# B3zaleel/draco-sharp

Hardware: AMD Instinct MI355X
Metric: decoded_meshes_per_sec (higher is better)
Workload: dtype int32

## Files before the change

draco-sharp_amd/csrc/dsa_kernels.h:

```cpp
#pragma once
#include <hip/hip_runtime.h>
#include <stdint.h>

#include "dsa_common.h"
#include "dsa_locate.h"
#include "dsa_needs.h"
#ifdef DSA_EXPERIMENTS
#include "dsa_lanes.h"
#else
#define LN_FLAG_SYMBOLS 1u
#define LN_FLAG_PREDICT 2u
#define LN_FLAG_OCT 8u
namespace dsa { namespace lanes {
__device__ __forceinline__ bool ln_sym_eligible(const AttrDesc &, const MeshLayout &, uint32_t, uint32_t) { return false; }
__device__ __forceinline__ bool ln_oct_eligible(const AttrDesc &, uint32_t) { return false; }
} }
#endif

#ifndef DSA_CHAIN_PRIO
#define DSA_CHAIN_PRIO 3
#endif

namespace dsa {

// ... 1376 lines not shown
        }
      }
      bool went_left = false;
      if (!went_right) {
        if (bits & 4u) {
          if (bits & 8u) { --sp; TPROF(5); break; }
          corner = lc;
          went_left = true;
        } else {
          if (bits & 8u) { corner = rc; went_right = true; }
          else {
            if (sp >= stack_cap) TR_FAIL(304);
            if (lane == 0) { stack[sp - 1] = lc; stack[sp] = rc; }
            ++sp;
            TPROF(5);
            break;
          }
        }
      }
      if (went_right && have2) { have_rec = true; have_state = true; c_v = c2_v; c_rc = c2_rc; c_lc = c2_lc; c_bits = c2_bits; }
      else if (have_kids && went_right) { have_rec = true; c_v = kr_v; c_rc = kr_rc; c_lc = kr_lc; }
      else if (have_kids && went_left) { have_rec = true; c_v = kl_v; c_rc = kl_rc; c_lc = kl_lc; }
      have2 = false;
      TPROF(5);
    }
    if (failed) break;
  }
  if (failed) return;
  if (lane == 0 && !position) { if (count != expect) fail(D, ST_INVALID, 305); }
  if (lane == 0 && position) {
    D->num_entries = count;
    D->dbg[5] = n_fail; D->dbg[6] = (uint32_t)(clk() - t_start);
    D->dbg[16] = (uint32_t)r_start; D->dbg[17] = (uint32_t)(realclk() - r_start);
    D->dbg[7] = n_run; D->dbg[8] = n_run_faces; D->dbg[9] = n_scalar; D->dbg[3] = n_fast;
#ifdef DSA_TRAV_PROFILE
    for (int i = 0; i < 5; ++i) D->dbg[10 + (i < 3 ? i : i + 5)] = (uint32_t)(tp_acc[i] >> 4);
    D->dbg[0] = (uint32_t)(tp_acc[5] >> 4); D->dbg[1] = np_fast_hit; D->dbg[2] = np_dep; D->dbg[4] = np_head; D->dbg[13] = np_hist; D->dbg[14] = np_lin; D->dbg[15] = np_hand;
    D->dbg[16] = np_pairs1; D->dbg[17] = np_pairs2;
#endif
    if (count != expect) fail(D, ST_INVALID, 305);
  }
  if ((fuse_operands & 1u) && count == expect) {
    WAIT_VM0();
    __threadfence_block();
    uint32_t *para = io.para;
    for (uint32_t p0 = 0; p0 < count; p0 += 4 * WAVE) {
      uint32_t en[4], ep[4], eo[4];
#pragma unroll
      for (int u = 0; u < 4; ++u) {
        const uint32_t p = p0 + u * WAVE + lane;
        para_operands_flat<CP>(p < count ? p : 0u, frec, d2c, v2d, F, NV, en[u], ep[u], eo[u]);
      }
#pragma unroll
      for (int u = 0; u < 4; ++u) {
        const uint32_t p = p0 + u * WAVE + lane;
        if (p < count) { Triple t; t.a = en[u]; t.b = ep[u]; t.c = eo[u]; *(Triple *)(para + 3 * (size_t)p) = t; }
      }
    }
  }
  if (position && !D->seam_fast && count == expect && NV) {
    WAIT_VM0();
    __threadfence_block();
    const uint32_t *vrank = (const uint32_t *)(arena + L.vrank);
    const uint32_t na = uni(D->num_attributes), npts = uni(D->num_points);
    for (uint32_t v0 = 0; v0 < NV; v0 += 4 * WAVE) {
      int32_t e[4];
      uint32_t point[4];
#pragma unroll
      for (int u = 0; u < 4; ++u) {
        const uint32_t v = v0 + u * WAVE + lane, vc = v < NV ? v : NV - 1;
        e[u] = v < NV ? v2d[vc] : -1;
        point[u] = vrank[vc];
      }
#pragma unroll
      for (int u = 0; u < 4; ++u)
        if (e[u] >= 0 && point[u] < npts)
          for (uint32_t ai = 0; ai < na; ++ai) ((uint32_t *)(arena + L.map[ai]))[point[u]] = (uint32_t)e[u];
    }
  }
#undef TR_FAIL
#undef VISIT_SCALAR
#undef TPROF
#undef TCOUNT
#undef TADD
#undef fA_before
#undef fB_before
#undef fR_before
#undef fL_before
#undef fLA_before
#undef flA
#undef flB
#undef TR_MARKS
}

__global__ __launch_bounds__(WAVE) void k_traverse(uint8_t *arena, const MeshLayout *layouts, MeshDesc *descs, uint32_t n, uint32_t fuse_operands) {
  __shared__ unsigned long long sh_tf[TR_SLOTS], sh_tv[TR_SLOTS];
  __shared__ uint32_t sh_hist[TR_HIST_WORDS];
  for (uint32_t i = threadIdx.x; i < TR_SLOTS; i += WAVE) { sh_tf[i] = 0; sh_tv[i] = 0; }
  if (threadIdx.x < TR_HIST_WORDS) sh_hist[threadIdx.x] = 0;
  __syncthreads();
  __builtin_amdgcn_s_setprio(DSA_CHAIN_PRIO);
  const uint32_t mesh = blockIdx.x;
  if (mesh >= n) return;
  if (status_of(&descs[mesh]) != ST_OK) return;
  const TravIO io = trav_position(arena, layouts[mesh], &descs[mesh]);
  if (layouts[mesh].rec_compact) traverse_wave<true>(arena, layouts[mesh], &descs[mesh], io, fuse_operands, sh_tf, sh_tv, sh_hist);
  else traverse_wave<false>(arena, layouts[mesh], &descs[mesh], io, fuse_operands, sh_tf, sh_tv, sh_hist);
}

extern __shared__ __attribute__((aligned(16))) uint32_t sh_chain[];
__global__ __launch_bounds__(WAVE, 8) void k_chain(uint8_t *arena, const MeshLayout *layouts, MeshDesc *descs, uint32_t n, uint32_t fuse_operands) {
  uint32_t *sh = sh_chain;
  static_assert(CN_LDS_WORDS * 4 >= 2 * TR_SLOTS * 8 + TR_HIST_WORDS * 4, "the traversal's tables reuse the connectivity's LDS");
  __builtin_amdgcn_s_setprio(DSA_CHAIN_PRIO);
  const uint32_t mesh = blockIdx.x;
  if (mesh >= n) return;
  const MeshLayout &L = layouts[mesh];
  MeshDesc *D = &descs[mesh];
  const bool compact = uni(L.rec_compact) != 0;
  uint32_t *sh_rec = sh + CN_STAGE * 8, *sh_win = sh_rec + CN_REC_BLOCKS * 64 * 2, *sh_ctx = sh_win + CN_WIN;
  if (!compact) connectivity_wave<false, false>(arena, L, D, sh, sh_rec, sh_win, sh_ctx);
  else if (uni((uint32_t)D->traversal_type) == 2u) connectivity_wave<true, true>(arena, L, D, sh, sh_rec, sh_win, sh_ctx);
  else connectivity_wave<true, false>(arena, L, D, sh, sh_rec, sh_win, sh_ctx);
  __builtin_amdgcn_fence(__ATOMIC_SEQ_CST, "agent");
  __syncthreads();
  unsigned long long *sh_tf = (unsigned long long *)sh, *sh_tv = sh_tf + TR_SLOTS;
  uint32_t *sh_hist = sh + 2 * TR_SLOTS * 2;
  for (uint32_t i = threadIdx.x; i < TR_SLOTS; i += WAVE) { sh_tf[i] = 0; sh_tv[i] = 0; }
  if (threadIdx.x < TR_HIST_WORDS) sh_hist[threadIdx.x] = 0;
  __syncthreads();
  if (status_of(D) != ST_OK) return;
  const TravIO io = trav_position(arena, L, D);
  if (compact) traverse_wave<true>(arena, L, D, io, fuse_operands, sh_tf, sh_tv, sh_hist);
  else traverse_wave<false>(arena, L, D, io, fuse_operands, sh_tf, sh_tv, sh_hist);
  if ((fuse_operands & 1u) && (fuse_operands & 8u) && status_of(D) == ST_OK) {
    const uint32_t na = uni(D->num_attributes);
    for (uint32_t ai = 0; ai < na && ai < DSA_MAX_ATT; ++ai) late_handoff(arena, L, D, ai, PW_FLAG | LATE_HANDOFF, 2u);
  }
}



__device__ __forceinline__ void rans_decode_wave(MeshDesc *D, const uint8_t *stream, uint32_t stream_len, const AttrDesc &a, uint32_t num_values,
                                 uint32_t *out, uint32_t *lds_cum, uint32_t *symtab) {
  const uint32_t lane = lane_id();
  const uint32_t nsym = symtab ? a.num_distinct : a.num_symbols;
  const uint32_t P = a.precision_bits, precision = 1u << P, l_base = precision * 4;
  if (lane == 0) {
    Rd r(stream, stream_len, a.off_table);
    if (symtab) {
      uint32_t k = 0;
      bool ok = true;
      for (uint32_t i = 0; i < a.num_symbols && ok; ++i) {
        const uint32_t pd = r.u8(), token = pd & 3u;
        if (token == 3u) { const uint32_t offset = pd >> 2; if (i + offset >= a.num_symbols) ok = false; i += offset; }
        else {
          uint32_t pr = pd >> 2;
          for (uint32_t j = 0; j < token; ++j) pr |= r.u8() << (8 * (j + 1) - 2);
          if (pr) { if (k >= nsym) ok = false; else { lds_cum[k] = pr; symtab[k] = i; ++k; } }
        }
      }
      if (!ok || !r.ok || k != nsym) fail(D, ST_INVALID, 400);
    } else if (!read_prob_table(r, nsym, lds_cum)) fail(D, ST_INVALID, 400);
  }
  WAIT_VM0();
  __syncthreads();
  if (status_of(D) != ST_OK) return;
  uint32_t carry = 0;
  for (uint32_t b0 = 0; b0 < nsym; b0 += WAVE) {
    uint32_t i = b0 + lane;
    uint32_t pr = i < nsym ? lds_cum[i] : 0u;
    uint32_t tot;
    uint32_t ex = wave_excl_scan(pr, &tot);
    if (i < nsym) lds_cum[i] = carry + ex;
    carry += tot;
  }
  if (carry != precision) { if (lane == 0) fail(D, ST_INVALID, 401); return; }
  const uint32_t nblocks = (nsym + WAVE - 1) / WAVE;
  for (uint32_t i = nsym + lane; i < nblocks * WAVE + 1; i += WAVE) lds_cum[i] = precision;
  __syncthreads();
  uint32_t coarse = (lane < nblocks) ? lds_cum[lane * WAVE] : precision;
  uint32_t fine0 = lds_cum[lane];
  const uint8_t *buf = stream + a.off_rans;
  uint32_t x, off;
  {
    uint32_t st = 0, o = 0;
    bool ok = rans_init(buf, a.size_rans, l_base, &st, &o);
    if (!ok) { if (lane == 0) fail(D, ST_INVALID, 402); return; }
    x = uni(st); off = uni(o);
  }
  const uintptr_t base_addr = (uintptr_t)buf;
  const uint32_t mis = (uint32_t)(base_addr & 3u);
  const uint32_t *abuf = (const uint32_t *)(base_addr - mis);
  uint32_t chunk = 0xFFFFFFFFu, W = 0;
  const uint32_t mask = precision - 1;
  uint32_t mine = 0;
  for (uint32_t i = 0; i < num_values; ++i) {
    while (x < l_base && off > 0) {
      --off;
      uint32_t q = off + mis;
      uint32_t ch = q >> 8;
      if (ch != chunk) { chunk = ch; W = abuf[(size_t)ch * 64 + lane]; }
      uint32_t byte = (rdlane(W, (q & 255u) >> 2) >> ((q & 3u) * 8)) & 0xFFu;
      x = (x << 8) | byte;
    }
    uint32_t rem = x & mask;
    uint32_t s, cs, nx;
    if (nblocks == 1) {
      uint32_t j = (uint32_t)__popcll(__ballot(fine0 <= rem)) - 1u;
      cs = rdlane(fine0, j);
      nx = (j < 63) ? rdlane(fine0, j + 1) : precision;
      s = j;
    } else {
      uint32_t b = (uint32_t)__popcll(__ballot(coarse <= rem)) - 1u;
      uint32_t v = lds_cum[b * WAVE + lane];
      uint32_t j = (uint32_t)__popcll(__ballot(v <= rem)) - 1u;
      cs = rdlane(v, j);
      nx = (j < 63) ? rdlane(v, j + 1) : rdlane(coarse, b + 1);
      s = b * WAVE + j;
    }
    x = (nx - cs) * (x >> P) + rem - cs;
    if ((i & 63u) == lane) mine = s;
    if ((i & 63u) == 63u) out[i - 63u + lane] = mine;
  }
  uint32_t tail = num_values & 63u;
  if (tail && lane < tail) out[num_values - tail + lane] = mine;
  if (symtab) {
    WAIT_VM0();
    __syncthreads();
    for (uint32_t i = lane; i < num_values; i += WAVE) out[i] = symtab[out[i]];
  }
}

__device__ __forceinline__ void rans_decode_serial(MeshDesc *D, const uint8_t *stream, uint32_t stream_len, const AttrDesc &a, uint32_t num_values,
                                   uint32_t *out, uint32_t *cum ) {
  if (threadIdx.x != 0) return;
  const uint32_t nsym = a.num_symbols, P = a.precision_bits, precision = 1u << P, l_base = precision * 4;
  Rd r(stream, stream_len, a.off_table);
  if (!read_prob_table(r, nsym, cum)) { fail(D, ST_INVALID, 410); return; }
  uint32_t c = 0;
  for (uint32_t i = 0; i < nsym; ++i) { uint32_t pr = cum[i]; cum[i] = c; c += pr; if (c > precision) break; }
  if (c != precision) { fail(D, ST_INVALID, 411); return; }
  cum[nsym] = precision;
  const uint8_t *buf = stream + a.off_rans;
  uint32_t x, off;
  if (!rans_init(buf, a.size_rans, l_base, &x, &off)) { fail(D, ST_INVALID, 412); return; }
  for (uint32_t i = 0; i < num_values; ++i) {
    while (x < l_base && off > 0) x = (x << 8) | buf[--off];
    uint32_t rem = x & (precision - 1);
    uint32_t lo = 0, hi = nsym;
    while (hi - lo > 1) { uint32_t mid = (lo + hi) >> 1; if (cum[mid] <= rem) lo = mid; else hi = mid; }
    uint32_t cs = cum[lo];
    x = (cum[lo + 1] - cs) * (x >> P) + rem - cs;
    out[i] = lo;
  }
}

typedef uint32_t v32u __attribute__((ext_vector_type(32)));

#define SYM_EARLY_FUSE 0x400u
__device__ __forceinline__ void predict_wave(uint8_t *arena, const MeshLayout &L, MeshDesc *D, uint32_t ai, uint32_t phase, uint32_t flags);
__device__ __forceinline__ void predict_wrap_attribute(uint8_t *arena, const MeshLayout &L, MeshDesc *D, uint32_t ai, uint32_t phase, uint32_t flags);
__device__ __forceinline__ void finalize_attribute(uint8_t *arena, const MeshLayout &L, const MeshDesc *D, uint32_t ai, uint32_t phase, uint32_t flags, uint32_t tid, uint32_t stride);
__device__ __forceinline__ void early_tail(uint8_t *arena, const MeshLayout &L, MeshDesc *D, uint32_t ai, uint32_t flags) {
  if (!(flags & SYM_EARLY_FUSE) || D->general) return;
  const AttrDesc &a = D->att[ai];
  if (att_is_late(a)) return;
  WAIT_VM0();
  __threadfence_block();
  __syncthreads();
  if (status_of(D) != ST_OK) return;
  predict_wrap_attribute(arena, L, D, ai, 0u, flags);
  predict_wave(arena, L, D, ai, 0u, flags);
  WAIT_VM0();
  __threadfence_block();
  __syncthreads();
  if (status_of(D) != ST_OK) return;
  finalize_attribute(arena, L, D, ai, 0u, flags, lane_id(), WAVE);
  if (lane_id() == 0) D->att[ai].early_done = 1;
}

__device__ __forceinline__ void late_handoff(uint8_t *arena, const MeshLayout &L, MeshDesc *D, uint32_t ai, uint32_t flags, uint32_t bit) {
  if (!(flags & LATE_HANDOFF) || D->general) return;
  AttrDesc &a = D->att[ai];
  if (!wrap_fast_ok(a, flags) || !att_is_late(a) || att_behind_tables(a) || a.pred_kind != 1) return;
  __builtin_amdgcn_fence(__ATOMIC_RELEASE, "agent");
  __syncthreads();
  uint32_t old = 0;
  if (lane_id() == 0) old = __hip_atomic_fetch_or(&a.late_ready, bit, __ATOMIC_ACQ_REL, __HIP_MEMORY_SCOPE_AGENT);
  old = uni(old);
  if (!(old & (3u ^ bit))) return;
  __builtin_amdgcn_fence(__ATOMIC_ACQUIRE, "agent");
  if (status_of(D) != ST_OK) return;
  predict_wrap_attribute(arena, L, D, ai, 1u, flags);
  WAIT_VM0();
  __syncthreads();
  if (lane_id() == 0) a.late_ready = 7u;
}

#define REG_ATTR 0
#define REG_TAGS 1
#define REG_VLIST 2
#define REG_SCRATCH_BYTES (4096u * 6u + REG_MAX_SYMS * 4u)
template <int MODE>
__device__ __forceinline__ void reg_decode_stream(uint8_t *arena, const MeshLayout &L, MeshDesc *D, uint32_t ai, uint32_t flags) {
  constexpr bool TAGS = MODE == REG_TAGS, VLIST = MODE == REG_VLIST;
  AttrDesc &a = D->att[VLIST ? 0u : ai];
  uint8_t *scratch;
  uint32_t st_off_table = a.off_table, st_off_rans = a.off_rans, st_size_rans = a.size_rans, st_nsym = a.num_symbols;
  uint32_t st_values = a.num_entries * (TAGS ? 1u : (uint32_t)a.nc_portable);
  uint32_t *out = (uint32_t *)(arena + L.work[VLIST ? 0u : ai]);
  if (VLIST) {
    st_values = D->val_count[ai];
    if (st_values == 0 || D->val_prec[ai] != 12 || D->val_nsym[ai] > 64) return;
    if ((uint64_t)L.rec_compact * 16ull * D->num_faces < 6ull * REG_SCRATCH_BYTES) return;
    st_off_table = D->val_off_table[ai]; st_off_rans = D->val_off_rans[ai]; st_size_rans = D->val_size_rans[ai]; st_nsym = D->val_nsym[ai];
    uint32_t before = 0;
    for (uint32_t k = 0; k < ai; ++k) before += D->val_count[k];
    if ((uint64_t)before + st_values > 3ull * D->num_faces) return;
    out = (uint32_t *)(arena + L.faces) + before;
    scratch = arena + L.frec + (size_t)ai * REG_SCRATCH_BYTES;
  } else if (TAGS) {
    if (a.source != SRC_TAGGED || a.tags_done || a.num_symbols > LOC_MAX_TAGS || a.num_distinct <= 1 || a.num_entries == 0) return;
    const uint64_t slots = ((uint64_t)a.num_entries * 4 + 15) & ~15ull;
    if ((uint64_t)L.work_cap[ai] * 4 < slots + REG_SCRATCH_BYTES) return;
    scratch = arena + L.work[ai] + slots;
  } else {
    if (lanes::ln_sym_eligible(a, L, ai, flags)) return;
    if (sym_filtered(a, flags)) return;
    if (!sym_reg_eligible(a, L, ai)) return;
    scratch = arena + L.out[ai];
  }
  const uint8_t *stream = arena + L.stream;
  uint32_t *slot_tab = (uint32_t *)scratch;
  uint16_t *slot_sym = (uint16_t *)(scratch + 4096 * 4);
  uint32_t *lds = (uint32_t *)(scratch + 4096 * 6);
  const uint32_t lane = lane_id();
  const uint32_t nsym = uni(st_nsym);
  const uint32_t num_values = uni(st_values);
  if (num_values == 0) return;
  if (lane == 0) {
    Rd r(stream, L.stream_len, st_off_table);
    if (!read_prob_table(r, nsym, lds)) fail(D, ST_INVALID, 400);
  }
  __syncthreads();
  if (status_of(D) != ST_OK) return;
  uint32_t carry = 0, one_at = DSA_INVALID;
  bool over = false;
  for (uint32_t b0 = 0; b0 < REG_MAX_SYMS; b0 += WAVE) {
    uint32_t i = b0 + lane;
    uint32_t pr = i < nsym ? lds[i] : 0u;
    if (pr > 4095) { over = true; one_at = i; }
    uint32_t tot;
    uint32_t ex = wave_excl_scan(pr, &tot);
    lds[i] = (pr << 12) | ((carry + ex) & 4095u);
    carry += tot;
    if (carry > 4096) over = true;
  }
  if (VLIST && carry == 4096 && __ballot(over)) {
    uint32_t st = 0, o = 0;
    if (!rans_init(stream + st_off_rans, st_size_rans, 16384, &st, &o)) { if (lane == 0) fail(D, ST_INVALID, 402); return; }
    const uint32_t one = (uint32_t)__builtin_ctzll(__ballot(one_at != DSA_INVALID));
    const uint32_t sym = rdlane(one_at, one);
    for (uint32_t i = lane; i < num_values; i += WAVE) out[i] = sym;
    WAIT_VM0();
    __syncthreads();
    if (lane == 0) atomicOr(&D->val_lists_done, 1u << ai);
    return;
  }
  if (__ballot(over) || carry != 4096) { if (lane == 0) fail(D, carry != 4096 ? ST_INVALID : ST_NOTIMPL, 401); return; }
  __syncthreads();
  for (uint32_t sy = lane; sy < nsym; sy += WAVE) {
    const uint32_t e = lds[sy], f = e >> 12, c = e & 4095u;
    for (uint32_t j = 0; j < f; ++j) { slot_tab[c + j] = f | (j << 16); slot_sym[c + j] = (uint16_t)sy; }
  }
  WAIT_VM0();
  __syncthreads();
  v32u tab_lo, tab_hi;
#pragma unroll
  for (int k = 0; k < 32; ++k) { tab_lo[k] = slot_tab[k * WAVE + lane]; tab_hi[k] = slot_tab[(k + 32) * WAVE + lane]; }
  const uint8_t *buf = stream + st_off_rans;
  uint32_t x, off;
  {
    uint32_t st = 0, o = 0;
    bool ok = rans_init(buf, st_size_rans, 16384, &st, &o);
    if (!ok) { if (lane == 0) fail(D, ST_INVALID, 402); return; }
    x = uni(st); off = uni(o);
  }
  const uint32_t mis = (uint32_t)((L.stream + st_off_rans) & 3u);
  const uint32_t *abuf = (const uint32_t *)(arena + (L.stream + st_off_rans - mis));
  uint32_t chunk = 0x7FFFFFFFu, W = 0;
  uint32_t mine = 0;
  WAIT_VM0();
  uint64_t P = (uint64_t)x << 32;
  uint32_t rc = 0;
  uint32_t dl = 0;
  bool exhausted = false;
  for (uint32_t i0 = 0; i0 < num_values; i0 += WAVE) {
    const uint32_t cnt = uni(num_values - i0 < WAVE ? num_values - i0 : WAVE);
    uint32_t j = 0;
    while (j < cnt) {
      if (!exhausted) {
        {
          uint32_t k6, va, vf;
          uint32_t js = uni(j);
          asm volatile(
              " s_getpc_b64 s[22:23]\n"
              "Lupc%=:\n"
              " s_mul_i32 %[k6], %[j], Lus1_%=-Lus0_%=\n"
              " s_add_u32 s22, s22, Lus0_%=-Lupc%=\n"
              " s_addc_u32 s23, s23, 0\n"
              " s_add_u32 s22, s22, %[k6]\n"
              " s_addc_u32 s23, s23, 0\n"
              " s_set_gpr_idx_on s22, gpr_idx(SRC1)\n"
              " s_setpc_b64 s[22:23]\n"
              ".irp J,0,1,2,3,4,5,6,7,8,9,10,11,12,13,14,15,16,17,18,19,20,21,22,23,24,25,26,27,28,29,30,31,32,33,34,35,36,37,38,39,40,41,42,43,44,45,46,47,48,49,50,51,52,53,54,55,56,57,58,59,60,61,62,63\n"
              "Lus\\J\\()_%=:\n"
              " s_cmpk_lt_u32 s21, 0x4000\n"
              " s_cbranch_scc1 Lur\\J\\()_%=\n"
              "Lok\\J\\()_%=:\n"
              " s_bfe_u32 %[k6], s21, 0x60006\n"
              " s_set_gpr_idx_idx %[k6]\n"
              " v_lshrrev_b32_e64 %[vf], 12, s21\n"
              " v_mul_u32_u24_sdwa %[va], %[vf], v16 dst_sel:DWORD dst_unused:UNUSED_PAD src0_sel:DWORD src1_sel:WORD_0\n"
              " v_add_u32_sdwa %[va], %[va], v16 dst_sel:DWORD dst_unused:UNUSED_PAD src0_sel:DWORD src1_sel:WORD_1\n"
              " v_writelane_b32 %[mine], s21, \\J\n"
              " v_readlane_b32 s21, %[va], s21\n"
              ".endr\n"
              " s_movk_i32 %[j], 64\n"
              " s_branch Luend%=\n"
              ".irp J,0,1,2,3,4,5,6,7,8,9,10,11,12,13,14,15,16,17,18,19,20,21,22,23,24,25,26,27,28,29,30,31,32,33,34,35,36,37,38,39,40,41,42,43,44,45,46,47,48,49,50,51,52,53,54,55,56,57,58,59,60,61,62,63\n"
              "Lur\\J\\()_%=:\n"
              " s_sub_u32 %[rc], %[rc], 1\n"
              " s_cbranch_scc1 Lue\\J\\()_%=\n"
              " s_lshl_b64 s[20:21], s[20:21], 8\n"
              " s_cmpk_lt_u32 s21, 0x4000\n"
              " s_cbranch_scc0 Lok\\J\\()_%=\n"
              " s_branch Lur\\J\\()_%=\n"
              "Lue\\J\\()_%=:\n"
              " s_cmp_lt_u32 %[off], 4\n"
              " s_cbranch_scc1 Lsl\\J\\()_%=\n"
              " s_sub_u32 %[dl], %[dl], 1\n"
              " s_cbranch_scc1 Lsl\\J\\()_%=\n"
              " v_readlane_b32 s20, %[W], %[dl]\n"
              " s_sub_u32 %[off], %[off], 4\n"
              " s_mov_b32 %[rc], 3\n"
              " s_lshl_b64 s[20:21], s[20:21], 8\n"
              " s_cmpk_lt_u32 s21, 0x4000\n"
              " s_cbranch_scc0 Lok\\J\\()_%=\n"
              " s_branch Lur\\J\\()_%=\n"
              "Lsl\\J\\()_%=:\n"
              " s_movk_i32 %[j], \\J\n"
              " s_branch Luempty%=\n"
              ".endr\n"
              "Luempty%=:\n"
              " s_mov_b32 %[rc], 0\n"
              "Luend%=:\n"
              " s_set_gpr_idx_off\n"
              : "+{s[20:21]}"(P), [rc] "+s"(rc), [j] "+s"(js), [mine] "+v"(mine), [k6] "=&s"(k6), [va] "=&v"(va), [vf] "=&v"(vf),
                [off] "+s"(off), [dl] "+s"(dl)
              : "{v[16:47]}"(tab_lo), "{v[48:79]}"(tab_hi), [W] "v"(W)
              : "vcc", "scc", "s22", "s23");
          j = js;
        }
        if (j < cnt) {
          if (off == 0) exhausted = true;
          else {
            const uint32_t end = off + mis;
            const uint32_t d = (end - 1) >> 2, r = end - 4 * d, ch = d >> 6;
            if (ch != chunk) { chunk = ch; W = abuf[(size_t)ch * 64 + lane]; WAIT_VM0(); }
            const uint32_t res = rdlane(W, d & 63u) << (8 * (4 - r));
            rc = uni(r < off ? r : off);
            off -= rc;
            dl = uni(d & 63u);
            P = (P & 0xFFFFFFFF00000000ull) | res;
          }
        }
      } else {
        const uint32_t xs = uni((uint32_t)(P >> 32));
        mine = (lane == j) ? xs : mine;
        const uint32_t k5 = (xs >> 6) & 31u, l6 = xs & 63u;
        const uint32_t e0 = rdlane(tab_lo[k5], l6), e1 = rdlane(tab_hi[k5], l6);
        const uint32_t e = (xs & 2048u) ? e1 : e0;
        P = (uint64_t)((e & 0xFFFFu) * (xs >> 12) + (e >> 16)) << 32;
        ++j;
      }
    }
    if (lane < cnt) out[i0 + lane] = mine;
  }
  WAIT_VM0();
  __syncthreads();
  if (VLIST) {
    for (uint32_t i = lane; i < num_values; i += WAVE) out[i] = slot_sym[out[i] & 4095u];
    WAIT_VM0();
    __syncthreads();
    if (lane == 0) atomicOr(&D->val_lists_done, 1u << ai);
    return;
  }
  if (TAGS) {
    uint8_t *tags = arena + L.out[ai];
    uint64_t bits = 0;
    uint32_t worst = 0;
    const uint32_t nc = a.nc_portable;
    for (uint32_t i = lane; i < num_values; i += WAVE) {
      const uint32_t v = slot_sym[out[i] & 4095u];
      tags[i] = (uint8_t)v;
      bits += (uint64_t)v * nc;
      worst = v > worst ? v : worst;
    }
    for (int d = 32; d >= 1; d >>= 1) {
      bits += ((uint64_t)(uint32_t)__shfl_xor((int)(uint32_t)(bits >> 32), d, WAVE) << 32) | (uint32_t)__shfl_xor((int)(uint32_t)bits, d, WAVE);
      const uint32_t w2 = (uint32_t)__shfl_xor((int)worst, d, WAVE);
      worst = w2 > worst ? w2 : worst;
    }
    WAIT_VM0();
    __syncthreads();
    if (lane == 0) { a.table = (bits & 0x00FFFFFFFFFFFFFFull) | ((uint64_t)(worst > 255u ? 255u : worst) << 56); a.tags_done = 1; }
    return;
  }
  const bool positive = a.have_scheme && (a.pred_transform == 2 || a.pred_transform == 3);
  for (uint32_t i = lane; i < num_values; i += WAVE) {
    uint32_t v = slot_sym[out[i] & 4095u];
    out[i] = positive ? v : ((v & 1u) ? (uint32_t)(-(int32_t)(v >> 1) - 1) : (v >> 1));
  }
  early_tail(arena, L, D, ai, flags);
  late_handoff(arena, L, D, ai, flags, 1u);
}

__global__ __launch_bounds__(WAVE, 6) void k_symbols_reg(uint8_t *arena, const MeshLayout *layouts, MeshDesc *descs, uint32_t n, uint32_t flags) {
  uint32_t mesh = blockIdx.x, ai = blockIdx.y;
  if (mesh >= n) return;
  MeshDesc *D = &descs[mesh];
  if (D->status != ST_OK || D->general || ai >= D->num_attributes) return;
  reg_decode_stream<REG_ATTR>(arena, layouts[mesh], D, ai, flags);
}
__global__ __launch_bounds__(WAVE, 6) void k_tags(uint8_t *arena, const MeshLayout *layouts, MeshDesc *descs, uint32_t n) {
  uint32_t mesh = blockIdx.x;
  if (mesh >= n) return;
  MeshDesc *D = &descs[mesh];
  if (D->status != ST_OK || D->general || !D->values_pending || D->resume_att >= D->num_attributes) return;
  if (D->values_pending == 2) return;
  reg_decode_stream<REG_TAGS>(arena, layouts[mesh], D, D->resume_att, 0u);
}
__global__ __launch_bounds__(WAVE, 6) void k_valence_lists(uint8_t *arena, const MeshLayout *layouts, MeshDesc *descs, uint32_t n) {
  uint32_t mesh = blockIdx.x, c = blockIdx.y;
  if (mesh >= n) return;
  MeshDesc *D = &descs[mesh];
  if (D->status != ST_OK || D->general || D->encoder_type == 0 || D->traversal_type != 2) return;
  reg_decode_stream<REG_VLIST>(arena, layouts[mesh], D, c, 0u);
}


__global__ __launch_bounds__(WAVE) void k_symbols_wide(uint8_t *arena, const MeshLayout *layouts, MeshDesc *descs, uint32_t n, uint32_t flags) {
  const uint32_t mesh = blockIdx.x, ai = blockIdx.y;
  if (mesh >= n) return;
  MeshDesc *D = &descs[mesh];
  if (D->status != ST_OK || D->general || ai >= D->num_attributes) return;
  const MeshLayout &L = layouts[mesh];
  const AttrDesc &a = D->att[ai];
  if (a.source == SRC_BYTES) return;
  if (lanes::ln_sym_eligible(a, L, ai, flags)) return;
  if (sym_filtered(a, flags)) return;
  if (!sym_wide_eligible(a, L, ai)) return;
  const uint32_t lane = lane_id();
  const uint32_t num_values = a.num_entries * a.nc_portable;
  if (num_values == 0) return;
  const uint8_t *stream = arena + L.stream;
  const uint32_t stream_len = L.stream_len;
  uint32_t *out = (uint32_t *)(arena + L.work[ai]);
  const bool compact = a.num_symbols > SYM_MAX_LDS;
  const uint32_t nsym = compact ? a.num_distinct : a.num_symbols;
  uint32_t *symtab = compact ? (uint32_t *)(arena + a.table) : nullptr;
  uint32_t *gtab = compact ? symtab + nsym : (uint32_t *)(arena + L.out[ai]);
  const uint32_t P = a.precision_bits, precision = 1u << P, l_base = precision * 4;
  if (lane == 0) {
    Rd r(stream, stream_len, a.off_table);
    uint32_t k = 0;
    bool ok = true;
    for (uint32_t i = 0; i < a.num_symbols && ok; ++i) {
      const uint32_t pd = r.u8(), token = pd & 3u;
      if (token == 3u) {
        const uint32_t offset = pd >> 2;
        if (i + offset >= a.num_symbols) ok = false;
        if (!compact) for (uint32_t j = 0; j <= offset && i + j < a.num_symbols; ++j) gtab[i + j] = 0;
        i += offset;
      } else {
        uint32_t pr = pd >> 2;
        for (uint32_t j = 0; j < token; ++j) pr |= r.u8() << (8 * (j + 1) - 2);
        if (compact) { if (pr) { if (k >= nsym) ok = false; else { gtab[k] = pr; symtab[k] = i; ++k; } } }
        else gtab[i] = pr;
      }
    }
    if (!ok || !r.ok || (compact && k != nsym)) fail(D, ST_INVALID, 400);
    WAIT_VM0();
    __threadfence_block();
  }
  __syncthreads();
  if (status_of(D) != ST_OK) return;
  uint32_t carry = 0;
  for (uint32_t b0 = 0; b0 < nsym; b0 += WAVE) {
    const uint32_t i = b0 + lane;
    const uint32_t pr = i < nsym ? gtab[i] : 0u;
    uint32_t tot;
    const uint32_t ex = wave_excl_scan(pr, &tot);
    if (i < nsym) gtab[i] = carry + ex;
    carry += tot;
  }
  if (carry != precision) { if (lane == 0) fail(D, ST_INVALID, 401); return; }
  if (lane == 0) gtab[nsym] = precision;
  WAIT_VM0();
  __threadfence_block();
  __syncthreads();
  const uint32_t nblocks = (nsym + WAVE - 1) / WAVE;
  const bool hand = uni(P) <= 15u;
  v32u tab;
#pragma unroll
  for (int r = 0; r < 32; ++r) {
    const uint32_t i = (uint32_t)r * WAVE + lane;
    const uint32_t c0 = i < nsym ? gtab[i] : 0x1FFFFu, c1 = i < nsym ? gtab[i + 1] : 0x1FFFFu;
    tab[r] = (i < nsym && c0 < 0x10000u && !(hand && c0 >= precision)) ? (hand ? ((c0 << 16) | (c1 - c0)) : (c0 | ((c1 - c0) << 16))) : 0xFFFFFFFFu;
  }
  const uint32_t coarse = lane < nblocks ? gtab[lane * WAVE] : 0xFFFFFFFFu;
  const uint8_t *buf = stream + a.off_rans;
  uint32_t x, off;
  {
    uint32_t st = 0, o = 0;
    const bool ok = rans_init(buf, a.size_rans, l_base, &st, &o);
    if (!ok) { if (lane == 0) fail(D, ST_INVALID, 402); return; }
    x = uni(st); off = uni(o);
  }
  const uintptr_t base_addr = (uintptr_t)buf;
  const uint32_t mis = (uint32_t)(base_addr & 3u);
  const uint32_t *abuf = (const uint32_t *)(base_addr - mis);
  uint32_t chunk = 0xFFFFFFFFu, W = 0;
  const uint32_t mask = precision - 1;
  uint32_t mine = 0;
  if (hand) {
    uint64_t PR = (uint64_t)x << 32;
    uint32_t rc = 0, dl = 0;
    bool exhausted = false;
    const uint32_t lb = uni(l_base), mk = uni(mask), pb = uni(P);
    uint32_t best = 0;
#pragma unroll
    for (int r = 0; r < 32; ++r) {
      const uint32_t w = tab[r], k = w == 0xFFFFFFFFu ? 0u : (((w & 0xFFFFu) << 11) | (uint32_t)(31 - r) << 6 | (63u - lane));
      best = k > best ? k : best;
    }
    for (int d = 32; d >= 1; d >>= 1) { const uint32_t o = (uint32_t)__shfl_xor((int)best, d, WAVE); best = o > best ? o : best; }
    const uint32_t idom = uni((31u - ((best >> 6) & 31u)) * WAVE + (63u - (best & 63u)));
    const uint32_t fdom = uni(best >> 11), cdom = uni(gtab[idom]), tdom = uni(idom + WAVE);
    WAIT_VM0();
    for (uint32_t i0 = 0; i0 < num_values; i0 += WAVE) {
      const uint32_t cnt = uni(num_values - i0 < WAVE ? num_values - i0 : WAVE);
      uint32_t j = 0;
      while (j < cnt) {
        if (!exhausted) {
          {
            uint32_t k6, rem, key, bb, q, t, jj, e, f, tmp;
            uint32_t js = uni(j);
            rc = uni(rc); off = uni(off); dl = uni(dl);
            PR = ((uint64_t)uni((uint32_t)(PR >> 32)) << 32) | uni((uint32_t)PR);
            asm volatile(
                " s_getpc_b64 s[22:23]\n"
                "Lwpc%=:\n"
                " s_mul_i32 %[k6], %[j], Lws1_%=-Lws0_%=\n"
                " s_add_u32 s22, s22, Lws0_%=-Lwpc%=\n"
                " s_addc_u32 s23, s23, 0\n"
                " s_add_u32 s22, s22, %[k6]\n"
                " s_addc_u32 s23, s23, 0\n"
                " s_set_gpr_idx_on s22, gpr_idx(SRC1)\n"
                " s_setpc_b64 s[22:23]\n"
                ".irp J,0,1,2,3,4,5,6,7,8,9,10,11,12,13,14,15,16,17,18,19,20,21,22,23,24,25,26,27,28,29,30,31,32,33,34,35,36,37,38,39,40,41,42,43,44,45,46,47,48,49,50,51,52,53,54,55,56,57,58,59,60,61,62,63\n"
                "Lws\\J\\()_%=:\n"
                " s_cmp_lt_u32 s21, %[lb]\n"
                " s_cbranch_scc1 Lwr\\J\\()_%=\n"
                "Lwk\\J\\()_%=:\n"
                " s_and_b32 %[rem], s21, %[mk]\n"
                " s_sub_u32 %[e], %[rem], %[cdom]\n"
                " s_cmp_lt_u32 %[e], %[fdom]\n"
                " s_cbranch_scc0 Lwq\\J\\()_%=\n"
                " s_lshr_b32 %[q], s21, %[pb]\n"
                " s_mul_i32 %[q], %[q], %[fdom]\n"
                " v_writelane_b32 %[mine], %[tdom], \\J\n"
                " s_add_u32 s21, %[q], %[e]\n"
                "Lwn\\J\\()_%=:\n"
                ".endr\n"
                " s_movk_i32 %[j], 64\n"
                " s_branch Lwend%=\n"
                ".irp J,0,1,2,3,4,5,6,7,8,9,10,11,12,13,14,15,16,17,18,19,20,21,22,23,24,25,26,27,28,29,30,31,32,33,34,35,36,37,38,39,40,41,42,43,44,45,46,47,48,49,50,51,52,53,54,55,56,57,58,59,60,61,62,63\n"
                "Lwq\\J\\()_%=:\n"
                " v_cmp_le_u32_e64 vcc, %[coarse], %[rem]\n"
                " s_pack_ll_b32_b16 %[key], 0xffff, %[rem]\n"
                " s_lshr_b32 %[q], s21, %[pb]\n"
                " s_bcnt1_i32_b64 %[bb], vcc\n"
                " s_set_gpr_idx_idx %[bb]\n"
                " s_lshl_b32 %[t], %[bb], 6\n"
                " v_or_b32_e32 %[tmp], 0, v15\n"
                " v_cmp_le_u32_e64 vcc, %[tmp], %[key]\n"
                " s_bcnt1_i32_b64 %[jj], vcc\n"
                " s_sub_u32 %[jj], %[jj], 1\n"
                " v_readlane_b32 %[e], %[tmp], %[jj]\n"
                " s_add_u32 %[t], %[t], %[jj]\n"
                " v_writelane_b32 %[mine], %[t], \\J\n"
                " s_and_b32 %[f], %[e], 0xffff\n"
                " s_lshr_b32 %[e], %[e], 16\n"
                " s_mul_i32 %[q], %[q], %[f]\n"
                " s_sub_u32 %[rem], %[rem], %[e]\n"
                " s_add_u32 s21, %[q], %[rem]\n"
                " s_branch Lwn\\J\\()_%=\n"
                ".endr\n"
                ".irp J,0,1,2,3,4,5,6,7,8,9,10,11,12,13,14,15,16,17,18,19,20,21,22,23,24,25,26,27,28,29,30,31,32,33,34,35,36,37,38,39,40,41,42,43,44,45,46,47,48,49,50,51,52,53,54,55,56,57,58,59,60,61,62,63\n"
                "Lwr\\J\\()_%=:\n"
                " s_sub_u32 %[rc], %[rc], 1\n"
                " s_cbranch_scc1 Lwe\\J\\()_%=\n"
                " s_lshl_b64 s[20:21], s[20:21], 8\n"
                " s_cmp_lt_u32 s21, %[lb]\n"
                " s_cbranch_scc0 Lwk\\J\\()_%=\n"
                " s_branch Lwr\\J\\()_%=\n"
                "Lwe\\J\\()_%=:\n"
                " s_cmp_lt_u32 %[off], 4\n"
                " s_cbranch_scc1 Lwl\\J\\()_%=\n"
                " s_sub_u32 %[dl], %[dl], 1\n"
                " s_cbranch_scc1 Lwl\\J\\()_%=\n"
                " v_readlane_b32 s20, %[W], %[dl]\n"
                " s_sub_u32 %[off], %[off], 4\n"
                " s_mov_b32 %[rc], 3\n"
                " s_lshl_b64 s[20:21], s[20:21], 8\n"
                " s_cmp_lt_u32 s21, %[lb]\n"
                " s_cbranch_scc0 Lwk\\J\\()_%=\n"
                " s_branch Lwr\\J\\()_%=\n"
                "Lwl\\J\\()_%=:\n"
                " s_movk_i32 %[j], \\J\n"
                " s_branch Lwempty%=\n"
                ".endr\n"
                "Lwempty%=:\n"
                " s_mov_b32 %[rc], 0\n"
                "Lwend%=:\n"
                " s_set_gpr_idx_off\n"
                : "+{s[20:21]}"(PR), [rc] "+s"(rc), [j] "+s"(js), [mine] "+v"(mine), [k6] "=&s"(k6), [rem] "=&s"(rem), [key] "=&s"(key), [bb] "=&s"(bb),
                  [q] "=&s"(q), [t] "=&s"(t), [jj] "=&s"(jj), [e] "=&s"(e), [f] "=&s"(f), [tmp] "=&v"(tmp), [off] "+s"(off), [dl] "+s"(dl)
                : "{v[16:47]}"(tab), [W] "v"(W), [coarse] "v"(coarse), [lb] "s"(lb), [mk] "s"(mk), [pb] "s"(pb), [cdom] "s"(cdom), [fdom] "s"(fdom), [tdom] "s"(tdom)
                : "vcc", "scc", "s22", "s23");
            j = js;
          }
          if (j < cnt) {
            if (off == 0) exhausted = true;
            else {
              const uint32_t end = off + mis;
              const uint32_t d = (end - 1) >> 2, r = end - 4 * d, ch = d >> 6;
              if (ch != chunk) { chunk = ch; W = abuf[(size_t)ch * 64 + lane]; WAIT_VM0(); }
              const uint32_t res = uni(rdlane(W, d & 63u) << (8 * (4 - r)));
              rc = uni(r < off ? r : off);
              off -= rc;
              dl = uni(d & 63u);
              PR = (PR & 0xFFFFFFFF00000000ull) | res;
            }
          }
        } else {
          const uint32_t xs = uni((uint32_t)(PR >> 32)), rem = xs & mk;
          const uint32_t b = uni((uint32_t)__popcll(__ballot(coarse <= rem)) - 1u);
          const uint32_t v = tab[b];
          const uint32_t jx = uni((uint32_t)__popcll(__ballot(v <= ((rem << 16) | 0xFFFFu))) - 1u);
          const uint32_t e = rdlane(v, jx);
          mine = (lane == j) ? (b + 1u) * WAVE + jx : mine;
          PR = (uint64_t)uni((e & 0xFFFFu) * (xs >> pb) + rem - (e >> 16)) << 32;
          ++j;
        }
      }
      if (lane < cnt) out[i0 + lane] = mine - WAVE;
    }
  } else {
  uint32_t res = 0, rc = 0;
  for (uint32_t i = 0; i < num_values; ++i) {
    while (x < l_base) {
      if (rc == 0) {
        if (off == 0) break;
        const uint32_t end = off + mis;
        const uint32_t d = (end - 1) >> 2, r = end - 4 * d, ch = d >> 6;
        if (ch != chunk) { chunk = ch; W = abuf[(size_t)ch * 64 + lane]; }
        res = rdlane(W, d & 63u) << (8 * (4 - r));
        rc = uni(r < off ? r : off);
        off -= rc;
      }
      x = (x << 8) | (res >> 24);
      res <<= 8;
      --rc;
    }
    const uint32_t rem = x & mask;
    const uint32_t b = uni((uint32_t)__popcll(__ballot(coarse <= rem)) - 1u);
    const uint32_t v = tab[b];
    const uint32_t j = (uint32_t)__popcll(__ballot((v & 0xFFFFu) <= rem && v != 0xFFFFFFFFu)) - 1u;
    const uint32_t e = rdlane(v, j);
    x = (e >> 16) * (x >> P) + rem - (e & 0xFFFFu);
    mine = (i & 63u) == lane ? b * WAVE + j : mine;
    if ((i & 63u) == 63u) out[i - 63u + lane] = mine;
  }
  const uint32_t tail = num_values & 63u;
  if (tail && lane < tail) out[num_values - tail + lane] = mine;
  }
  WAIT_VM0();
  __threadfence_block();
  __syncthreads();
  const bool positive = a.have_scheme && (a.pred_transform == 2 || a.pred_transform == 3);
  for (uint32_t i = lane; i < num_values; i += WAVE) {
    uint32_t v = out[i];
    if (compact) v = symtab[v];
    out[i] = positive ? v : ((v & 1u) ? (uint32_t)(-(int32_t)(v >> 1) - 1) : (v >> 1));
  }
}

template <int TIER>
__device__ __forceinline__ void symbols_tier_item(uint8_t *arena, const MeshLayout *layouts, MeshDesc *descs, uint32_t mesh, uint32_t ai, uint32_t flags, uint32_t *lds_cum) {
  MeshDesc *D = &descs[mesh];
  if (D->status != ST_OK || D->general || ai >= D->num_attributes) return;
  const MeshLayout &L = layouts[mesh];
  const AttrDesc &a = D->att[ai];
  if (a.source == SRC_BYTES) return;
  if (lanes::ln_sym_eligible(a, L, ai, flags)) return;
  if (sym_filtered(a, flags)) return;
  const bool compact = sym_tier_compact(a);
  if (sym_tier_of(a, L, ai, flags) != TIER) return;
  const uint8_t *s = arena + L.stream;
  uint32_t *work = (uint32_t *)(arena + L.work[ai]);
  const uint32_t lane = lane_id();
  const uint32_t nc = a.nc_portable;
  const uint32_t num_values = a.num_entries * nc;
  if (num_values == 0) return;
// ... 764 lines not shown
```

Measured before the change: 109,100.

## Prefetch next rANS chunk and fuse symbol mapping into decode loop

The wave-serial rANS decoder now issues the load of the next (preceding) 256-byte stream chunk after each 64-value batch, so a later chunk switch can use the prefetched register instead of stalling on a global load. In attribute mode it also looks up the symbol table and applies the zigzag/sign transform for each batch and writes it one batch late, which removes the separate post-pass that re-read and re-wrote the output array. Timing stamps behind a compile flag are added for profiling. The prefetch assumes the stream is consumed backwards chunk by chunk, and the deferred write adds a little register pressure.

```diff
diff --git a/draco-sharp_amd/csrc/dsa_kernels.h b/draco-sharp_amd/csrc/dsa_kernels.h
--- a/draco-sharp_amd/csrc/dsa_kernels.h
+++ b/draco-sharp_amd/csrc/dsa_kernels.h
@@ -1702,11 +1702,23 @@
 #define REG_TAGS 1
 #define REG_VLIST 2
 #define REG_SCRATCH_BYTES (4096u * 6u + REG_MAX_SYMS * 4u)
+#ifdef DSA_SYM_STAMPS
+#define REG_STAMP_BEGIN() uint64_t st_t = clk()
+#define REG_STAMP(p) { const uint64_t t_ = clk(); if (ATTR && ai < 3 && lane_id() == 0) { const uint32_t k_ = 3u * (p) + ai; \
+    ((uint16_t *)D->dbg)[k_ < 6 ? 20 + k_ : 30 + k_] = (uint16_t)((t_ - st_t) >> 10 > 65535 ? 65535 : (t_ - st_t) >> 10); } st_t = t_; }
+#else
+#define REG_STAMP_BEGIN()
+#define REG_STAMP(p)
+#endif
+__device__ __forceinline__ uint32_t reg_final_symbol(uint32_t v, bool positive) {
+  return positive ? v : ((v & 1u) ? (uint32_t)(-(int32_t)(v >> 1) - 1) : (v >> 1));
+}
 template <int MODE>
 __device__ __forceinline__ void reg_decode_stream(uint8_t *arena, const MeshLayout &L, MeshDesc *D, uint32_t ai, uint32_t flags) {
-  constexpr bool TAGS = MODE == REG_TAGS, VLIST = MODE == REG_VLIST;
+  constexpr bool TAGS = MODE == REG_TAGS, VLIST = MODE == REG_VLIST, ATTR = MODE == REG_ATTR;
   AttrDesc &a = D->att[VLIST ? 0u : ai];
   uint8_t *scratch;
+  REG_STAMP_BEGIN();
   uint32_t st_off_table = a.off_table, st_off_rans = a.off_rans, st_size_rans = a.size_rans, st_nsym = a.num_symbols;
   uint32_t st_values = a.num_entries * (TAGS ? 1u : (uint32_t)a.nc_portable);
   uint32_t *out = (uint32_t *)(arena + L.work[VLIST ? 0u : ai]);
@@ -1790,8 +1802,12 @@
   const uint32_t mis = (uint32_t)((L.stream + st_off_rans) & 3u);
   const uint32_t *abuf = (const uint32_t *)(arena + (L.stream + st_off_rans - mis));
   uint32_t chunk = 0x7FFFFFFFu, W = 0;
+  uint32_t next_chunk = 0x7FFFFFFFu, Wn = 0;
   uint32_t mine = 0;
+  uint32_t pend = 0;
+  const bool positive = ATTR && a.have_scheme && (a.pred_transform == 2 || a.pred_transform == 3);
   WAIT_VM0();
+  REG_STAMP(0);
   uint64_t P = (uint64_t)x << 32;
   uint32_t rc = 0;
   uint32_t dl = 0;
@@ -1868,7 +1884,11 @@
           else {
             const uint32_t end = off + mis;
             const uint32_t d = (end - 1) >> 2, r = end - 4 * d, ch = d >> 6;
-            if (ch != chunk) { chunk = ch; W = abuf[(size_t)ch * 64 + lane]; WAIT_VM0(); }
+            if (ch != chunk) {
+              if (next_chunk == ch) W = Wn;
+              else { W = abuf[(size_t)ch * 64 + lane]; WAIT_VM0(); }
+              chunk = ch;
+            }
             const uint32_t res = rdlane(W, d & 63u) << (8 * (4 - r));
             rc = uni(r < off ? r : off);
             off -= rc;
@@ -1886,7 +1906,15 @@
         ++j;
       }
     }
-    if (lane < cnt) out[i0 + lane] = mine;
+    if (ATTR) { if (i0) out[i0 - WAVE + lane] = reg_final_symbol(pend, positive); }
+    else if (lane < cnt) out[i0 + lane] = mine;
+    if (chunk != 0x7FFFFFFFu && chunk != 0 && next_chunk != chunk - 1) { next_chunk = chunk - 1; Wn = abuf[next_chunk * 64u + lane]; }
+    if (ATTR) pend = slot_sym[mine & 4095u];
+  }
+  REG_STAMP(1);
+  if (ATTR) {
+    const uint32_t last = (num_values - 1) & ~(WAVE - 1u);
+    if (lane < num_values - last) out[last + lane] = reg_final_symbol(pend, positive);
   }
   WAIT_VM0();
   __syncthreads();
@@ -1918,11 +1946,7 @@
     if (lane == 0) { a.table = (bits & 0x00FFFFFFFFFFFFFFull) | ((uint64_t)(worst > 255u ? 255u : worst) << 56); a.tags_done = 1; }
     return;
   }
-  const bool positive = a.have_scheme && (a.pred_transform == 2 || a.pred_transform == 3);
-  for (uint32_t i = lane; i < num_values; i += WAVE) {
-    uint32_t v = slot_sym[out[i] & 4095u];
-    out[i] = positive ? v : ((v & 1u) ? (uint32_t)(-(int32_t)(v >> 1) - 1) : (v >> 1));
-  }
+  REG_STAMP(2);
   early_tail(arena, L, D, ai, flags);
   late_handoff(arena, L, D, ai, flags, 1u);
 }
```

New measurement: 112,000 (median of 6 runs). 2.6% higher.
